# flanglet/kanzi-cpp

Measured on AMD Instinct MI355X. Metric: encode+decode MB/s on the synthetic stand-in for silesia.tar (bit-exact), higher is better.
Workload: dtype u8

## Files before the change

kanzi-cpp_amd/csrc/bwt_fwd.hip:

```cpp
#include "common.hpp"
#include "stages.hpp"
#include "bwt_common.hpp"

#include <cstdlib>
#include <cstring>
#include <algorithm>
#include <cmath>
#include "prims.hpp"
#include <chrono>
#include <vector>

namespace knz {

constexpr u32 SM_TS = 1792;
constexpr u32 SM_WIN = 2048;
constexpr u32 SM_G = 256;
constexpr u32 MED_CAP = 8192;
constexpr u32 MED_LO_CAP = 2048;
constexpr u32 SUPER_CAP = 8192;
constexpr int GATHER_THREADS = 512;
constexpr u32 GATHER_ROWS = 16;
static_assert(MED_CAP <= GATHER_ROWS * GATHER_THREADS, "k_bwt_f_gather_desc judges a medium group from one batch of loads");
constexpr u32 LARGE_OS_MIN = 1000000;
constexpr u32 NO_BIT = 0x7FFFFFFFu;
// ... 23 lines not shown

enum FwdCounter : u32 {
    CNT_SMALL_LEFT = 0,
    CNT_MED = 1,
    CNT_LARGE = 2,
    CNT_LARGE_MEMBERS = 3,
    CNT_RUN = 4,
    CNT_RUN_MEMBERS = 5,
    CNT_RUN_LONGEST = 6,
    CNT_SUPER = 7,
    CNT_RUNS = 8,
    CNT_MED_LO = 9,
    CNT_STAT_SMALL = 10,
    CNT_STAT_SMALL_GROUPS = 11,
    CNT_STAT_MED = 12,
    CNT_TIED = 13,
    CNT_PROBE_CAND = 14,
    CNT_LINKED = 14,
    CNT_LINK_TIED = 15,
    CNT_STAT_MED_GROUPS = 16,
    CNT_STAT_UNSPLIT = 17,
    CNT_STAT_UNSPLIT_MEMBERS = 18,
    CNT_STAT_MAJ = 19,
    CNT_STAT_MAJ_MEMBERS = 20,
    CNT_STAT_ASLEEP = 21,
    CNT_STAT_ASLEEP_MEMBERS = 22,
    CNT_RUN_TILES = 23,
    CNT_ROUND_SLOTS = 24,
    CNT_GAP_CLASSES = 25,
    CNT_GAP_MEMBERS = 26,
// ... 284 lines not shown
    __shared__ u32 inclAll[256];
    const int sgm = blockIdx.x, ps = blockIdx.y;
    const int tid = (int)threadIdx.x;
    u32* h = L.histAll + ((size_t)ps * L.nSeg + sgm) * 256;
    const u32 c = h[tid];
    u32 tot;
    const u32 incl = prims::sc_block_incl<prims::SCAN_SUM_EXCL>(c, wsum, &tot);
    inclAll[tid] = incl;
    __syncthreads();
    const bool last = ps + 1 == P;
    const u32 b0 = last ? base[sgm] : cbase[sgm];
    h[tid] = b0 + (tid ? inclAll[tid - 1] : 0u);
    if (last) gapStart[(size_t)sgm * 256 + tid] = b0 + incl - members[(size_t)sgm * 256 + tid];
}

__global__ __launch_bounds__(256) void k_bwt_f_r0_fill(u64* __restrict__ keys, const u32* __restrict__ members, const u32* __restrict__ gapStart,
                                                       const u32* __restrict__ firstPos, int P, int pbits)
{
    const u32 sgm = blockIdx.y;
    for (u32 c = 0; c < 256u; c++) {
        const u32 m = members[sgm * 256u + c];
        if (m == 0u) continue;
        const u32 g0 = gapStart[sgm * 256u + c];
        const u64 key = (rep_key(c, P) << pbits) | (u64)firstPos[sgm * 256u + c];
        for (u32 i = blockIdx.x * 256u + threadIdx.x; i < m; i += gridDim.x * 256u) keys[g0 + i] = key;
    }
}

constexpr u32 R0F_ROWS = 8;
__global__ __launch_bounds__(256) void k_bwt_f_r0_flags(const u64* __restrict__ keys, const u32* __restrict__ base, int nBlocks, u32 total, int P, int pbits,
                                                        unsigned long long* __restrict__ gbits64)
{
    __shared__ int sBlk;
    const u32 a0 = blockIdx.x * (256u * R0F_ROWS);
    if (threadIdx.x == 0) sBlk = find_block(base, nBlocks, a0 < total ? a0 : (total ? total - 1 : 0));
    __syncthreads();
    u64 kr[R0F_ROWS], kl[R0F_ROWS];
#pragma unroll
    for (u32 r = 0; r < R0F_ROWS; r++) {
        const u32 a = a0 + r * 256u + threadIdx.x;
        kr[r] = (a < total) ? keys[a] : 0ull;
        kl[r] = ((threadIdx.x & 63) == 0 && a > 0 && a < total) ? keys[a - 1] : 0ull;
    }
    int b = sBlk;
    const u64 pm = (1ull << pbits) - 1ull;
#pragma unroll
    for (u32 r = 0; r < R0F_ROWS; r++) {
        const u32 a = a0 + r * 256u + threadIdx.x;
        if (a0 + r * 256u >= total) break;
        const u64 k = kr[r];
        const u32 klo = (u32)__shfl_up((int)(u32)k, 1u, 64), khi = (u32)__shfl_up((int)(u32)(k >> 32), 1u, 64);
// ... 72 lines not shown
    const u32 word = W.bw[w];
    const u32 m = word & lowmask;
    int si = m ? (int)(w * 32 + 31 - __clz((int)m)) : W.prevSet[w];
    if (si < 0 || (u32)si >= SM_TS) return false;
    const u32 m2 = word & ~lowmask;
    const u32 ei = m2 ? (w * 32 + (u32)__ffs((int)m2) - 1) : W.nextSet[w];
    if (ei == NO_BIT) return false;
    const u32 len = ei - (u32)si;
    if (len < 2 || len > SM_G) return false;
    s = (u32)si; e = ei;
    return true;
}

__global__ __launch_bounds__(256) void k_bwt_f_r0_place_text(BwtView bv, FwdView v, const u32* __restrict__ winLastIncl, const u32* __restrict__ winFirstInclRev, u32 nWin,
                                                             uint2* __restrict__ largeNext, const u64* __restrict__ keys, int nsym, int pbits, uint2* __restrict__ runList,
                                                             const u32* __restrict__ gapTab)
{
    __shared__ SmWindow W;
    __shared__ int sBlk;
    __shared__ ClassAgg A;
    __shared__ u32 sSA[SM_WIN];
    __shared__ u64 sK[SM_WIN];
    __shared__ u32 sNew[64];
    __shared__ u32 sAfterLocal;
    constexpr int E = (int)(SM_WIN / 256);
    constexpr u32 TSW = SM_TS / 32;
    const int tid = (int)threadIdx.x;
    const u32 win = blockIdx.x;
    const u32 slot0 = win * SM_TS;
    if (tid == 0) sBlk = find_block(v.base, v.nBlocks, slot0 < v.total ? slot0 : v.total - 1);
    agg_init(A);
    if (tid < 64) {
        sNew[tid] = 0;
        const u32 w = v.gbits[(slot0 >> 5) + (u32)tid];
        W.bw[tid] = w;
        int pm = w ? (tid * 32 + 31 - __clz((int)w)) : -1;
        u32 sm = w ? (u32)(tid * 32 + __ffs((int)w) - 1) : NO_BIT;
        for (int o = 1; o < 64; o <<= 1) {
            const int t = __shfl_up(pm, (unsigned)o, 64);
            if (tid >= o) pm = t > pm ? t : pm;
            const u32 u = (u32)__shfl_down((int)sm, (unsigned)o, 64);
            if (tid + o < 64) sm = u < sm ? u : sm;
        }
        int pex = __shfl_up(pm, 1u, 64);
        if (tid == 0) pex = -1;
// ... 1683 lines not shown
static_assert(RUN_COLS == 4 * 256 && RUN_CH == 256 && RUN_ROWS % 4 == 0, "the kernels below map columns and rows to 256 threads");
static inline size_t run_tile_slots(size_t maxRuns) { return 2 * (maxRuns / RUN_TILE + 2); }

struct RunTile { u32 k0, k1, a, slot; bool first, last, multi; };
__device__ __forceinline__ RunTile run_tile(const u32* __restrict__ tileStart, const u32* __restrict__ segStart, u32 nRuns, u32 t)
{
    RunTile r;
    r.k0 = tileStart[t]; r.k1 = tileStart[t + 1]; r.a = segStart[r.k0];
    r.first = r.k0 == r.a;
    r.last = r.k1 >= nRuns || segStart[r.k1] == r.k1;
    r.multi = !(r.first && r.last);
    r.slot = (r.k1 - r.k0 == RUN_TILE) ? 2u * ((r.k0 + RUN_TILE - 1) / RUN_TILE) : (r.k0 >= RUN_TILE ? 2u * ((r.k0 - 1) / RUN_TILE) + 1u : 1u);
    return r;
}

__global__ __launch_bounds__(256) void k_bwt_f_run_seg_marks(const u64* __restrict__ sKey, u32 nRuns, int kbits, u32* __restrict__ segMark)
{
    const u32 k = blockIdx.x * 256 + threadIdx.x;
    if (k >= nRuns) return;
    segMark[k] = (k > 0 && (sKey[k] >> kbits) == (sKey[k - 1] >> kbits)) ? 0u : k;
}

__global__ __launch_bounds__(256) void k_bwt_f_run_tile_marks(const u32* __restrict__ segStart, u32 nRuns, u32* __restrict__ tileMark)
{
    const u32 k = blockIdx.x * 256 + threadIdx.x;
    if (k >= nRuns) return;
    tileMark[k] = ((k - segStart[k]) % RUN_TILE == 0) ? 1u : 0u;
}

__global__ __launch_bounds__(256) void k_bwt_f_run_tile_starts(const u32* __restrict__ segStart, const u32* __restrict__ tileIdx, u32 nRuns, u32* __restrict__ tileStart)
{
    const u32 k = blockIdx.x * 256 + threadIdx.x;
    if (k >= nRuns) return;
    const bool mark = (k - segStart[k]) % RUN_TILE == 0;
    const u32 t = tileIdx[k];
// ... 52 lines not shown
    }
    u32 run[4];
#pragma unroll
    for (u32 c = 0; c < 4; c++) run[c] = above ? carry - P[c] : P[c] - A[c];
    for (u32 t = t0; t < nT; t++) {
        const RunTile T = run_tile(tileStart, segStart, nRuns, t);
        u32* row = colTab + (size_t)T.slot * RUN_COLS;
#pragma unroll
        for (u32 c = 0; c < 4; c++) { const u32 x = row[tid + 256 * c]; row[tid + 256 * c] = run[c]; run[c] += x; }
        if (T.last) break;
    }
}

__global__ __launch_bounds__(256) void k_bwt_f_run_emit(const u32* __restrict__ tileStart, const u32* __restrict__ segStart, const u32* __restrict__ rcnt,
                                                        const u32* __restrict__ moff, const u64* __restrict__ sKey, const u32* __restrict__ sE, u32 nRuns, u32 M,
                                                        const u32* __restrict__ nTilesDev, const u32* __restrict__ colTab, u32 nsym, int kbits, int hbits,
                                                        u64* __restrict__ keys, u32* __restrict__ vals, u32* __restrict__ Rout)
{
    __shared__ u32 cnt[RUN_ROWS][RUN_CH];
    __shared__ u32 colBase[RUN_CH];
    __shared__ u32 wsum[4];
    __shared__ u32 sLmax;
    const u32 t = blockIdx.x, tid = threadIdx.x;
    if (t >= *nTilesDev) return;
    const int lane = lane_id();
    const u32 wave = tid >> 6;
    const RunTile T = run_tile(tileStart, segStart, nRuns, t);
    const u32 nRows = (T.k1 - T.k0 + 63) / 64;
    const u32 segBase = moff[T.a];
    const u32 tileMembers = (T.k1 < nRuns ? moff[T.k1] : M) - moff[T.k0];
    const bool above = ((sKey[T.k0] >> kbits) & 1ull) != 0;
    const u64 hiAll = (1ull << hbits) - 1ull;
    u32 Lr[RUN_ROWS / 4], rowMax[RUN_ROWS / 4], e[RUN_ROWS / 4];
    u64 kb[RUN_ROWS / 4];
    u32 lmax = 0;
    if (tid == 0) sLmax = 0;
#pragma unroll
    for (u32 q = 0; q < RUN_ROWS / 4; q++) {
        const u32 k = T.k0 + (wave + 4 * q) * 64 + (u32)lane;
        Lr[q] = 0; e[q] = 0; kb[q] = 0;
        if (k < T.k1) {
            const u64 key = sKey[k];
            Lr[q] = rcnt[k] + nsym - 1u;
            if (Lr[q] > RUN_DIRECT_LMAX) Lr[q] = RUN_DIRECT_LMAX;
            e[q] = sE[k];
            kb[q] = ((key >> (kbits + 1)) << (hbits + kbits)) | (key & ((1ull << kbits) - 1ull));
        }
        rowMax[q] = wave_max(Lr[q]);
        lmax = rowMax[q] > lmax ? rowMax[q] : lmax;
    }
    __syncthreads();
    if (lane == 0) atomicMax(&sLmax, lmax);
    __syncthreads();
    const u32 Lmax = sLmax;
    u32 carry = 0;
    for (u32 c0 = nsym; c0 <= Lmax; c0 += RUN_CH) {
        for (u32 i = tid; i < nRows * RUN_CH; i += 256) (&cnt[0][0])[i] = 0;
        __syncthreads();
#pragma unroll
        for (u32 q = 0; q < RUN_ROWS / 4; q++)
            if (Lr[q] >= c0) atomicAdd(&cnt[wave + 4 * q][Lr[q] - c0 < RUN_CH ? Lr[q] - c0 : RUN_CH - 1], 1u);
// ... 21 lines not shown
            const u32 P = carry + prims::sc_block_incl<prims::SCAN_SUM_EXCL>(colRuns, wsum, &tot);
            colBase[tid] = above ? tileMembers - P : P - colRuns;
            carry += tot;
        }
        __syncthreads();
#pragma unroll
        for (u32 q = 0; q < RUN_ROWS / 4; q++) {
            const u32 row = wave + 4 * q;
            if (row >= nRows) break;
            const u32 Rend = rowMax[q] < c0 + RUN_CH - 1 ? rowMax[q] : c0 + RUN_CH - 1;
            for (u32 R = c0; R <= Rend; R++) {
                const bool alive = Lr[q] >= R;
                const unsigned long long m = __ballot(alive);
                const u32 j = segBase + colBase[R - c0] + cnt[row][R - c0] + (u32)__popcll(m & __lanemask_lt());
                if (alive && j < M) {
                    keys[j] = kb[q] | ((above ? hiAll - (u64)R : (u64)R) << kbits);
                    vals[j] = e[q] - R;
                    Rout[j] = R;
                }
            }
        }
        __syncthreads();
    }
}

__global__ __launch_bounds__(256) void k_bwt_f_run_flags(const u64* __restrict__ keys, u32 M, unsigned long long* __restrict__ bits64)
{
    const u32 j = blockIdx.x * 256 + threadIdx.x;
    const u64 k = (j < M) ? keys[j] : 0ull;
    u32 klo = (u32)__shfl_up((int)(u32)k, 1u, 64), khi = (u32)__shfl_up((int)(u32)(k >> 32), 1u, 64);
    u64 kp = ((u64)khi << 32) | klo;
    if ((threadIdx.x & 63) == 0 && j > 0 && j < M) kp = keys[j - 1];
    const bool f = (j >= M) || (j == 0) || (k != kp);
    const unsigned long long m = __ballot(f);
    if ((threadIdx.x & 63) == 0) bits64[j >> 6] = m;
}

__global__ __launch_bounds__(256) void k_bwt_f_run_place(FwdView v, const uint2* __restrict__ desc, const u32* __restrict__ loff, u32 M, int kbits, const u64* __restrict__ keys,
                                                         const u32* __restrict__ vals, const u32* __restrict__ bits, const u32* __restrict__ winLastIncl,
                                                         const u32* __restrict__ winFirstInclRev, u32 nWin, uint2* __restrict__ largeNext, const u32* __restrict__ memberR,
                                                         u32* __restrict__ ovr, u32* __restrict__ rtbits, const u32* __restrict__ lbase, int allLabels)
{
    __shared__ SmWindow W;
    __shared__ ClassAgg A;
    const int tid = (int)threadIdx.x;
    const u32 jb = blockIdx.x * 256u;
    const u32 win = jb / SM_WIN, j0 = win * SM_WIN;
    agg_init(A);
    if (tid < 64) {
        const u32 w = bits[(j0 >> 5) + (u32)tid];
        W.bw[tid] = w;
        int pm = w ? (tid * 32 + 31 - __clz((int)w)) : -1;
        u32 sm = w ? (u32)(tid * 32 + __ffs((int)w) - 1) : NO_BIT;
        for (int o = 1; o < 64; o <<= 1) {
            const int t = __shfl_up(pm, (unsigned)o, 64);
            if (tid >= o) pm = t > pm ? t : pm;
            const u32 u = (u32)__shfl_down((int)sm, (unsigned)o, 64);
            if (tid + o < 64) sm = u < sm ? u : sm;
        }
        int pex = __shfl_up(pm, 1u, 64);
        if (tid == 0) pex = -1;
        u32 sex = (u32)__shfl_down((int)sm, 1u, 64);
        if (tid == 63) sex = NO_BIT;
// ... 1 lines not shown
        W.nextSet[tid] = sex;
    }
    __syncthreads();
    const u32 j = jb + (u32)tid;
    u32 surv = 0, mySlot = 0, hLocal = 0, hSize = 0;
    int hKind = -1;
    bool setBit = false;
    if (j < M) {
        const u32 i = j - j0;
        const u32 w = i >> 5, bit = i & 31;
        const u32 lowmask = (bit == 31) ? 0xFFFFFFFFu : ((2u << bit) - 1u);
        const u32 word = W.bw[w];
        const u32 m = word & lowmask;
        const int si = m ? (int)(w * 32 + 31 - (u32)__clz((int)m)) : W.prevSet[w];
        const u32 nh = (si >= 0) ? j0 + (u32)si : (win ? winLastIncl[win - 1] : 0u);
        const u32 di = (u32)(keys[j] >> kbits);
        const u32 gs = desc[di].x, off = loff[di];
        const u32 gp = vals[j];
        mySlot = gs + (j - off);
        v.SA[mySlot] = gp;
        if (nh != off || allLabels) lab_set(v, gp, lbase[di], gs + (nh - off), gs);
        ovr[mySlot] = memberR[j];
        if (nh == j) {
            const u32 m2 = word & ~lowmask;
            const u32 ei = m2 ? (w * 32 + (u32)__ffs((int)m2) - 1) : W.nextSet[w];
            u32 nxt = (ei != NO_BIT) ? j0 + ei : ((win + 1 < nWin) ? winFirstInclRev[nWin - 2 - win] : M);
            if (nxt > M) nxt = M;
            setBit = (j != off);
            hSize = nxt - j;
            hKind = agg_note(A, hSize, false, surv, hLocal);
        }
    }
    if (__ballot(surv != 0) != 0 && (tid & 63) == 0) v.counters[CNT_SMALL_LEFT] = 1;
    __syncthreads();
    if (tid == 0) agg_reserve(A, v);
    __syncthreads();
    if (hKind >= 0) agg_write(A, v, hKind, hLocal, mySlot, hSize, largeNext, (uint2*)nullptr);
    const int lane = tid & 63;
    const bool live = j < M;
    const u32 s0 = (u32)__shfl((int)mySlot, 0, 64);
    const bool inLine = live && (mySlot == s0 + (u32)lane);
    const unsigned long long hm = __ballot(setBit && inLine), rm = __ballot(inLine);
    if (live && !inLine) {
        if (setBit) atomicOr(&v.gnew[mySlot >> 5], 1u << (mySlot & 31));
        atomicOr(&rtbits[mySlot >> 5], 1u << (mySlot & 31));
    }
    if (lane == 0) {
        const u32 w0 = s0 >> 5, sh = s0 & 31;
        for (int which = 0; which < 2; which++) {
            const unsigned long long mask = which ? rm : hm;
            u32* dst = which ? rtbits : v.gnew;
            if (mask == 0) continue;
            const u32 p0 = (u32)(mask << sh);
            const u32 p1 = sh ? (u32)(mask >> (32 - sh)) : (u32)(mask >> 32);
            const u32 p2 = sh ? (u32)(mask >> (64 - sh)) : 0u;
            if (p0) atomicOr(&dst[w0], p0);
            if (p1) atomicOr(&dst[w0 + 1], p1);
            if (p2) atomicOr(&dst[w0 + 2], p2);
        }
    }
}

__global__ __launch_bounds__(256) void k_bwt_f_merge_bits(u32* __restrict__ gbits, u32* __restrict__ gnew, u32 nWords)
{
    const u32 w = blockIdx.x * 256 + threadIdx.x;
    if (w >= nWords) return;
    const u32 x = gnew[w];
    if (x) { gbits[w] |= x; gnew[w] = 0; }
}

__global__ __launch_bounds__(256) void k_bwt_f_emit(BwtView v, const u32* __restrict__ base, const u8* __restrict__ ok, const u32* __restrict__ SA,
                                                    FwdView fv, u32* __restrict__ newLen)
{
    const int b = blockIdx.y;
// ... 210 lines not shown
};

struct FwdSort {
    hipStream_t s; const XfStage& st; u32* hp;
    const FwdTuning tune = fwd_tuning();
    BwtView bv; FwdView v; FwdScratch w; size_t maxTotal;
    prims::RsWs rs1;
    u32 total, medSlots, nTiles; int nsym, pbits, kbits;
    bool groupSleep = false;
    u32 h = 1; int cur = 0;
    u64 *keysFree, *keysFree2;
    bool medFuse = false;
    bool runDirect = false;
    bool gaps = false;
    u32 gapClasses = 0, keptOut = 0, scanRuns = 0, scanLongest = 0;
    u32 nMedLo = 0;
    u32 nRun, runElems, surv, nMed, nLarge, largeElems, survMembers;
    LinkPlan link; LinkTrial linkTr; std::chrono::steady_clock::time_point statT;
    int fetch(u32 first, u32 n) { return hipMemcpyAsync(hp + first, w.counters + first, 4 * (size_t)n, hipMemcpyDeviceToHost, s) == hipSuccess && hipStreamSynchronize(s) == hipSuccess ? 0 : -1; }
    void merge_bits() { hipLaunchKernelGGL(k_bwt_f_merge_bits, GRID1(total / 32 + 2), w.gbits, w.gnew, total / 32 + 2); }
    void enable_run_tiebits() { if (!v.rtbits) { hipMemsetAsync(w.rtbits, 0, 4 * w.gbitsWords, s); v.ovr = w.ovr; v.rtbits = w.rtbits; } }
    void compact_medium(uint2* dst, u32 at = 0, u32 atLo = 0)
    {
        KScope ks_("k_bwt_f_med_compact");
        hipLaunchKernelGGL(k_bwt_f_med_flags, GRID1(medSlots), w.medStage, medSlots, w.medFlags);
        prims::launch_scan<prims::SCAN_SUM_EXCL>(s, w.medFlags, w.medPrefix, 2 * (size_t)medSlots, nullptr, w.scanTmp, w.counters + CNT_MED);
        hipLaunchKernelGGL(k_bwt_f_med_compact, GRID1(medSlots), w.medStage, medSlots, w.medPrefix, dst, at, w.medIdxLo, atLo, w.medIdxHi, at - atLo, w.counters + CNT_MED_LO);
    }
    void bounds(u32 n, bool last, const u32* bits = nullptr, u32 len = 0, u32 wordsPerWin = 0)
    {
// ... 74 lines not shown
        hipLaunchKernelGGL(k_bwt_f_r0_bases, dim3((unsigned)rs.L.nSeg, (unsigned)nsym), dim3(256), 0, s, rs.L, w.base, w.cbase, nsym, w.gapMembers, w.gapStart);
        for (int pass = 0; pass < nsym; pass++) {
            if (pass == 0) {
                TextSrcKept src; src.src = bv.src; src.P = nsym; src.pbits = pbits; src.shift = pbits; src.members = w.gapMembers;
                prims::rs_launch_pass_os<u64, false>(s, rs, src, nullptr, kout, nullptr, (size_t)bv.VS, pass);
                prims::rs_launch_layout(s, rsC);
            } else if (pass + 1 < nsym) {
                prims::DigitOfKey<u64> src; src.keys = kin; src.shift = pbits + 8 * pass; src.mask = 255u;
                prims::rs_launch_pass_os<u64, false>(s, rsC, src, nullptr, kout, nullptr, (size_t)bv.VS, pass);
            } else {
                LastPassSrc src; src.keys = kin; src.shift = pbits + 8 * pass; src.mask = 255u; src.members = w.gapMembers; src.gapStart = w.gapStart; src.P = nsym; src.pbits = pbits;
                prims::rs_launch_pass_os<u64, false>(s, rsC, src, nullptr, kout, nullptr, (size_t)bv.VS, pass);
            }
            std::swap(kin, kout);
        }
        hipLaunchKernelGGL(k_bwt_f_r0_fill, dim3(128, (unsigned)st.nBlocks), dim3(256), 0, s, kin, w.gapMembers, w.gapStart, w.gapFirst, nsym, pbits);
        keysFree = kout; keysFree2 = kin;
    }
    void round0_sort()
    {
        const prims::RsWs rs = prims::rs_carve(w.rsMem, maxTotal, st.nBlocks + 1, w.base, st.nBlocks);
        rs1 = prims::rs_carve(w.rsMem, maxTotal, st.nBlocks + 1, w.seg2, 1);
        { KScope ks_("k_bwt_f_r0_layout"); prims::rs_launch_layout(s, rs); }
        u64* kin = w.keysA; u64* kout = w.keysB;
        const bool oneRead = one_read();
        if (gaps) { round0_sort_gaps(rs); return; }
        if (oneRead) {
            KScope ks_("k_bwt_f_r0_sort");
            hipLaunchKernelGGL(k_bwt_f_r0_counts, dim3((unsigned)rs.L.nSeg), dim3(256), 0, s, bv, w.base, w.byteHist, nsym, rs.L, (const u32*)nullptr);
            hipLaunchKernelGGL(prims::k_rs_digit_bases, dim3((unsigned)rs.L.nSeg, (unsigned)nsym), dim3(256), 0, s, rs.L);
        }
// ... 2 lines not shown
            else prims::rs_launch_pass<u64, false>(s, rs, src, nullptr, kout, nullptr, (size_t)bv.VS);
        };
        for (int pass = 0; pass < nsym; pass++) {
            KScope ks_("k_bwt_f_r0_sort");
            if (pass == 0) { TextSrc src; src.src = bv.src; src.P = nsym; src.pbits = pbits; src.shift = pbits; sortPass(src, pass); }
            else { prims::DigitOfKey<u64> src; src.keys = kin; src.shift = pbits + 8 * pass; src.mask = 255u; sortPass(src, pass); }
            std::swap(kin, kout);
        }
        keysFree = kout; keysFree2 = kin;
    }
    int round0_place()
    {
        hipMemsetAsync(w.gbits, 0xFF, 4 * w.gbitsWords, s); hipMemsetAsync(w.gnew, 0, 4 * w.gbitsWords, s);
        hipMemsetAsync(w.counters, 0, 4 * CNT_ROUND_SLOTS, s);
        { KScope ks_("k_bwt_f_r0_flags"); hipLaunchKernelGGL(k_bwt_f_r0_flags, dim3((total + 256 * R0F_ROWS - 1) / (256 * R0F_ROWS)), dim3(256), 0, s, keysFree2, w.base, st.nBlocks, total, nsym, pbits,
                                                             reinterpret_cast<unsigned long long*>(w.gbits)); }
        bounds(nTiles, true, w.gbits, total, SM_TS / 32);
        kbits = bits_for((u64)bv.VS + 2, 1);
        const bool runRound = (2 * kbits + 1) < 64 && !tune.noRunRound;
        { KScope ks_("k_bwt_f_r0_place");
          hipLaunchKernelGGL(k_bwt_f_r0_place_text, dim3(nTiles), dim3(256), 0, s, bv, v, w.t1, w.t3, nTiles, w.large[cur], keysFree2, nsym, pbits, runRound ? w.runList : (uint2*)nullptr,
                             gaps ? w.classTab : (const u32*)nullptr);
          merge_bits(); }
        if (fetch(0, CNT_ROUND_SLOTS)) return -1;
        nRun = hp[CNT_RUN]; runElems = hp[CNT_RUN_MEMBERS];
        return 0;
    }
    int run_fallback()
    {
        { KScope ks_("k_bwt_f_run_fallback"); hipLaunchKernelGGL(k_bwt_f_run_fallback, GRID1(nRun), v, w.runList, nRun, w.med[cur], w.large[cur]); }
        nRun = 0; return fetch(0, CNT_ROUND_SLOTS);
    }
    int run_round()
    {
        if (nRun && ((u64)nRun > (1ull << (64 - (2 * kbits + 1))) || tune.runFallback) && run_fallback()) return -1;
        if (gaps) {
            if (nRun != gapClasses || runElems != keptOut) return -1;
            { KScope ks_("k_bwt_f_run_classes"); hipLaunchKernelGGL(k_bwt_f_run_classes, GRID1(nRun), bv, v, w.runList, nRun, w.classTab); }
            return run_round_sorted(scanRuns, scanLongest);
        }
// ... 12 lines not shown
        return run_round_sorted(hp[CNT_RUNS], hp[CNT_RUN_LONGEST]);
    }
    int run_round_sorted(const u32 nRuns, const u32 longest)
    {
        const int hbits = bits_for((u64)longest + 1, 1) + 1;
        const int rbits = bits_for(nRun, 0), idxBits = bits_for(nRuns, 1);
        if (nRuns == 0 || nRuns > w.maxRuns || rbits + hbits > 32 || idxBits + kbits + 1 + rbits > 64) return gaps ? -1 : run_fallback();
        { KScope ks_("k_bwt_f_large_prefix"); hipLaunchKernelGGL(k_bwt_f_large_prefix, dim3(1), dim3(1024), 0, s, w.runList, nRun, w.loff, w.base, st.nBlocks, w.lbase); }
        { KScope ks_("k_bwt_f_run_table"); hipLaunchKernelGGL(k_bwt_f_run_table, GRID1(nRuns), bv, v, w.runPos, nRuns, w.K, w.classTab, kbits, idxBits, w.runKeysA, w.runE, w.runL,
                                                              gaps ? w.runList : (const uint2*)nullptr, (u32)nsym); }
        const u64* rkSorted;
        { KScope ks_("k_bwt_f_sort_runs");
          rkSorted = sort_one_segment<u64, false>(nRuns, w.runKeysA, w.runKeysB, nullptr, nullptr, idxBits, idxBits + kbits + 1 + rbits) ? w.runKeysB : w.runKeysA; }
        { KScope ks_("k_bwt_f_run_sorted"); hipLaunchKernelGGL(k_bwt_f_run_sorted, GRID1(nRuns), rkSorted, nRuns, idxBits, w.runE, w.runL, (u32)nsym, w.sE, w.sKey, w.rcnt); }
        { KScope ks_("k_bwt_f_scan_sum"); prims::launch_scan<prims::SCAN_SUM_EXCL>(s, w.rcnt, w.moff, nRuns, nullptr, w.scanTmp); }
        u64* rk; u32* rv = w.valsA;
        runDirect = !tune.runSort && longest <= RUN_DIRECT_LMAX;
        if (runDirect) {
            KScope ks_("k_bwt_f_run_direct");
            u32* segStart = w.runPos; u32* tileIdx = w.runE;
            const u32 maxTiles = (u32)std::min<u64>((u64)nRuns, 2ull * nRun + nRuns / RUN_TILE + 1);
            hipLaunchKernelGGL(k_bwt_f_run_seg_marks, GRID1(nRuns), w.sKey, nRuns, kbits, segStart);
            prims::launch_scan<prims::SCAN_MAX_INCL>(s, segStart, segStart, nRuns, nullptr, w.scanTmp);
            hipLaunchKernelGGL(k_bwt_f_run_tile_marks, GRID1(nRuns), segStart, nRuns, tileIdx);
            prims::launch_scan<prims::SCAN_SUM_EXCL>(s, tileIdx, tileIdx, nRuns, nullptr, w.scanTmp, w.counters + CNT_RUN_TILES);
            hipLaunchKernelGGL(k_bwt_f_run_tile_starts, GRID1(nRuns), segStart, tileIdx, nRuns, w.runTileStart);
            if (nRuns > RUN_TILE) {
                hipLaunchKernelGGL(k_bwt_f_run_tile_counts, dim3(maxTiles), dim3(256), 0, s, w.runTileStart, segStart, w.rcnt, nRuns, w.counters + CNT_RUN_TILES, (u32)nsym, w.runColTab);
                hipLaunchKernelGGL(k_bwt_f_run_tile_scan, dim3(maxTiles), dim3(256), 0, s, w.runTileStart, segStart, w.sKey, nRuns, w.counters + CNT_RUN_TILES, (u32)nsym, kbits, w.runColTab);
            }
            rk = keysFree;
            hipLaunchKernelGGL(k_bwt_f_run_emit, dim3(maxTiles), dim3(256), 0, s, w.runTileStart, segStart, w.rcnt, w.moff, w.sKey, w.sE, nRuns, runElems, w.counters + CNT_RUN_TILES,
                               w.runColTab, (u32)nsym, kbits, hbits, rk, rv, w.valsB);
        } else {
            { KScope ks_("k_bwt_f_run_members"); hipLaunchKernelGGL(k_bwt_f_run_members, dim3((runElems + 2047) / 2048), dim3(256), 0, s, w.moff, nRuns, runElems, w.sKey, kbits, hbits,
                                                                    (u32)nsym, keysFree); }
            KScope ks_("k_bwt_f_sort_members");
            const int r = sort_one_segment<u64, false>(runElems, keysFree, keysFree2, nullptr, nullptr, 32, 32 + hbits + rbits);
            rk = r ? keysFree : keysFree2;
            hipLaunchKernelGGL(k_bwt_f_run_expand, GRID1(runElems), r ? keysFree2 : keysFree, runElems, w.sKey, w.sE, kbits, hbits, rk, rv, w.valsB);
        }
        u32* mbits = w.ebits; const u32 nWinM = (runElems + SM_WIN - 1) / SM_WIN;
        { KScope ks_("k_bwt_f_large_flags"); hipLaunchKernelGGL(k_bwt_f_run_flags, dim3(nWinM * (SM_WIN / 256)), dim3(256), 0, s, rk, runElems, reinterpret_cast<unsigned long long*>(mbits)); }
        bounds(nWinM, true, mbits, runElems, SM_WIN / 32);
        { KScope ks_("k_bwt_f_large_place");
          hipMemsetAsync(w.rtbits, 0, 4 * w.gbitsWords, s);
          hipLaunchKernelGGL(k_bwt_f_run_place, dim3((runElems + 255) / 256), dim3(256), 0, s, v, w.runList, w.loff, runElems, hbits + kbits, rk, rv, mbits, w.t1, w.t3, nWinM, w.large[cur],
                             w.valsB, w.ovr, w.rtbits, w.lbase, gaps ? 1 : 0);
          v.ovr = w.ovr; v.rtbits = w.rtbits; }
        { KScope ks_("k_bwt_f_merge_bits"); merge_bits(); }
        return 0;
    }
    int probe()
    {
        u32* probeCand = w.medFlags;
        compact_medium(w.med[cur]);
        { KScope ks_("k_bwt_f_probe"); hipLaunchKernelGGL(k_bwt_f_probe_scan, dim3(256), dim3(256), 0, s, v, w.med[cur], (u32)nsym, v.rtbits, probeCand); }
        if (fetch(0, CNT_ROUND_SLOTS)) return -1;
        surv = hp[CNT_SMALL_LEFT]; nMed = hp[CNT_MED]; nMedLo = hp[CNT_MED_LO]; nLarge = hp[CNT_LARGE]; largeElems = hp[CNT_LARGE_MEMBERS];
        if (const u32 nCand = hp[CNT_PROBE_CAND]) {
            enable_run_tiebits();
            hipMemsetAsync(w.counters, 0, 4 * CNT_PROBE_SLOTS, s);
            { KScope ks_("k_bwt_f_probe");
              hipLaunchKernelGGL(k_bwt_f_probe, dim3(std::min<u32>(nCand, 4096)), dim3(512), 0, s, bv, v, w.med[cur], probeCand, nCand, (u32)nsym, w.med[cur ^ 1], w.large[cur], w.ovr, w.rtbits);
              merge_bits(); }
            compact_medium(w.med[cur], nMed, nMedLo);
            if (fetch(0, CNT_MED_LO + 1)) return -1;
            surv |= hp[CNT_SMALL_LEFT]; nMed += hp[CNT_MED]; nMedLo += hp[CNT_MED_LO];
        }
        if (tune.stats) fprintf(stderr, "after round 0 (nsym %d, total %u): run groups %u (%u members); small left %u, medium %u, large %u (%u members); run members placed directly %u, sorted %u, kept out of the round-0 sort %u\n",
                                nsym, total, nRun, runElems, surv, nMed, nLarge, largeElems, (nRun && runDirect) ? runElems : 0u, (nRun && !runDirect) ? runElems : 0u, gaps ? keptOut : 0u);
        statT = std::chrono::steady_clock::now();
        return 0;
    }
    void link_step()
    {
        KScope ks_("k_bwt_f_link");
        u32* posflag = w.ebits; u32* linked = w.rbits; u32* rev = w.rcount; u32* sufRev = w.rprefix;
        const bool trial = link.mode == LinkPlan::TRIAL; linkTr.n = 0;
        if (trial) { linkTr.blk[linkTr.n++] = 0; if (st.nBlocks >= 5) linkTr.blk[linkTr.n++] = st.nBlocks / 2; if (st.nBlocks >= 3) linkTr.blk[linkTr.n++] = st.nBlocks - 1; }
        const u32 nW = total / 32 + 1;
        hipMemsetAsync(posflag, 0, 4 * (size_t)nW, s);
        hipMemsetAsync(linked, 0, 4 * ((size_t)nTiles * (SM_TS / 32) + 64), s);
        enable_run_tiebits();
        const u32 nTrial = (u32)std::min<u64>((u64)nTiles, ((u64)bv.VS + SM_TS - 1) / SM_TS + 2);
        const dim3 gridL(trial ? nTrial : nTiles, (unsigned)(linkTr.n ? linkTr.n : 1));
// ... 117 lines not shown
```

Measured before the change: 7424.

## Skip round-0 work inside gap interiors and emit run members directly into SA

Round-0 fill now writes keys only at the two margins of each large gap class. The flag and place kernels return early for workgroups that lie wholly inside a gap, clearing the gap's flag words instead of scanning keys. On the direct run path, the emit kernel now writes SA, ovr and a tie-flag byte straight to final slots, using string-mark and tie scans, rather than building keys and values. The place kernel is templated to find descriptors by binary search on loff. This removes full-key traffic and the run_flags pass, at the cost of extra scans, new kernels and more complex correctness conditions.

```diff
diff --git a/kanzi-cpp_amd/csrc/bwt_fwd.hip b/kanzi-cpp_amd/csrc/bwt_fwd.hip
--- a/kanzi-cpp_amd/csrc/bwt_fwd.hip
+++ b/kanzi-cpp_amd/csrc/bwt_fwd.hip
@@ -61,6 +61,7 @@
     CNT_STAT_SMALL = 10,
     CNT_STAT_SMALL_GROUPS = 11,
     CNT_STAT_MED = 12,
+    CNT_STAT_R0_SKIPPED = 12,
     CNT_TIED = 13,
     CNT_PROBE_CAND = 14,
     CNT_LINKED = 14,
@@ -375,27 +376,50 @@
     if (last) gapStart[(size_t)sgm * 256 + tid] = b0 + incl - members[(size_t)sgm * 256 + tid];
 }
 
+constexpr u32 R0F_ROWS = 8;
+constexpr u32 R0_GAP_MARGIN = 2048;
+static_assert(R0_GAP_MARGIN >= 256 * R0F_ROWS, "a workgroup of k_bwt_f_r0_flags that touches a gap's end must stay within the margin");
+static_assert(R0_GAP_MARGIN >= SM_WIN, "a window of k_bwt_f_r0_place_text that touches a gap's end must stay within the margin");
+
+__device__ __forceinline__ bool r0_inside_gap(const u32* __restrict__ members, const u32* __restrict__ gapStart, int b, u32 c, u32 a, u32 n)
+{
+    const u32 m = members[(u32)b * 256u + c];
+    if (m == 0u) return false;
+    const u32 g0 = gapStart[(u32)b * 256u + c];
+    return a > g0 && a - g0 < m && n <= m - (a - g0);
+}
+
 __global__ __launch_bounds__(256) void k_bwt_f_r0_fill(u64* __restrict__ keys, const u32* __restrict__ members, const u32* __restrict__ gapStart,
                                                        const u32* __restrict__ firstPos, int P, int pbits)
 {
-    const u32 sgm = blockIdx.y;
-    for (u32 c = 0; c < 256u; c++) {
-        const u32 m = members[sgm * 256u + c];
-        if (m == 0u) continue;
-        const u32 g0 = gapStart[sgm * 256u + c];
-        const u64 key = (rep_key(c, P) << pbits) | (u64)firstPos[sgm * 256u + c];
-        for (u32 i = blockIdx.x * 256u + threadIdx.x; i < m; i += gridDim.x * 256u) keys[g0 + i] = key;
-    }
-}
-
-constexpr u32 R0F_ROWS = 8;
+    const u32 sgm = blockIdx.y, c = blockIdx.x;
+    const u32 m = members[sgm * 256u + c];
+    if (m == 0u) return;
+    const u32 g0 = gapStart[sgm * 256u + c];
+    const u64 key = (rep_key(c, P) << pbits) | (u64)firstPos[sgm * 256u + c];
+    const bool whole = m <= 2u * R0_GAP_MARGIN;
+    const u32 cnt = whole ? m : 2u * R0_GAP_MARGIN;
+    for (u32 i = threadIdx.x; i < cnt; i += 256u) keys[g0 + ((whole || i < R0_GAP_MARGIN) ? i : m - 2u * R0_GAP_MARGIN + i)] = key;
+}
+
 __global__ __launch_bounds__(256) void k_bwt_f_r0_flags(const u64* __restrict__ keys, const u32* __restrict__ base, int nBlocks, u32 total, int P, int pbits,
-                                                        unsigned long long* __restrict__ gbits64)
+                                                        unsigned long long* __restrict__ gbits64, const u32* __restrict__ members, const u32* __restrict__ gapStart,
+                                                        u32* __restrict__ nSkipped)
 {
     __shared__ int sBlk;
+    __shared__ u32 sInside;
     const u32 a0 = blockIdx.x * (256u * R0F_ROWS);
-    if (threadIdx.x == 0) sBlk = find_block(base, nBlocks, a0 < total ? a0 : (total ? total - 1 : 0));
-    __syncthreads();
+    if (threadIdx.x == 0) { sBlk = find_block(base, nBlocks, a0 < total ? a0 : (total ? total - 1 : 0)); sInside = 0; }
+    __syncthreads();
+    if (members != nullptr) {
+        if (r0_inside_gap(members, gapStart, sBlk, threadIdx.x, a0, 256u * R0F_ROWS)) sInside = 1;
+        __syncthreads();
+        if (sInside) {
+            if (threadIdx.x < 256u * R0F_ROWS / 64u) gbits64[(a0 >> 6) + threadIdx.x] = 0ull;
+            if (nSkipped != nullptr && threadIdx.x == 0) atomicAdd(nSkipped, 1u);
+            return;
+        }
+    }
     u64 kr[R0F_ROWS], kl[R0F_ROWS];
 #pragma unroll
     for (u32 r = 0; r < R0F_ROWS; r++) {
@@ -498,7 +522,7 @@
 
 __global__ __launch_bounds__(256) void k_bwt_f_r0_place_text(BwtView bv, FwdView v, const u32* __restrict__ winLastIncl, const u32* __restrict__ winFirstInclRev, u32 nWin,
                                                              uint2* __restrict__ largeNext, const u64* __restrict__ keys, int nsym, int pbits, uint2* __restrict__ runList,
-                                                             const u32* __restrict__ gapTab)
+                                                             const u32* __restrict__ gapTab, const u32* __restrict__ gapMembers, const u32* __restrict__ gapStart)
 {
     __shared__ SmWindow W;
     __shared__ int sBlk;
@@ -507,12 +531,19 @@
     __shared__ u64 sK[SM_WIN];
     __shared__ u32 sNew[64];
     __shared__ u32 sAfterLocal;
+    __shared__ u32 sInside;
     constexpr int E = (int)(SM_WIN / 256);
     constexpr u32 TSW = SM_TS / 32;
     const int tid = (int)threadIdx.x;
     const u32 win = blockIdx.x;
     const u32 slot0 = win * SM_TS;
-    if (tid == 0) sBlk = find_block(v.base, v.nBlocks, slot0 < v.total ? slot0 : v.total - 1);
+    if (gapTab != nullptr) {
+        if (tid == 0) { sBlk = find_block(v.base, v.nBlocks, slot0 < v.total ? slot0 : v.total - 1); sInside = 0; }
+        __syncthreads();
+        if (r0_inside_gap(gapMembers, gapStart, sBlk, (u32)tid, slot0, SM_WIN)) sInside = 1;
+        __syncthreads();
+        if (sInside) return;
+    } else if (tid == 0) sBlk = find_block(v.base, v.nBlocks, slot0 < v.total ? slot0 : v.total - 1);
     agg_init(A);
     if (tid < 64) {
         sNew[tid] = 0;
@@ -2226,11 +2257,51 @@
     return r;
 }
 
-__global__ __launch_bounds__(256) void k_bwt_f_run_seg_marks(const u64* __restrict__ sKey, u32 nRuns, int kbits, u32* __restrict__ segMark)
+__global__ __launch_bounds__(256) void k_bwt_f_run_seg_marks(const u64* __restrict__ sKey, u32 nRuns, int kbits, u32* __restrict__ segMark, u32* __restrict__ strMark)
 {
     const u32 k = blockIdx.x * 256 + threadIdx.x;
     if (k >= nRuns) return;
-    segMark[k] = (k > 0 && (sKey[k] >> kbits) == (sKey[k - 1] >> kbits)) ? 0u : k;
+    const u64 key = sKey[k], prev = k > 0 ? sKey[k - 1] : 0ull;
+    segMark[k] = (k > 0 && (key >> kbits) == (prev >> kbits)) ? 0u : k;
+    strMark[k] = (k > 0 && key == prev) ? 0u : k;
+}
+
+constexpr int RUN_LBITS = 10;
+static_assert(RUN_DIRECT_LMAX < (1u << RUN_LBITS), "a run length of the direct path fits the low bits of tie[]");
+__global__ __launch_bounds__(256) void k_bwt_f_run_tie_marks(u32* __restrict__ tie, const u32* __restrict__ rcnt, u32 nRuns, u32 nsym)
+{
+    const u32 k = blockIdx.x * 256 + threadIdx.x;
+    if (k >= nRuns) return;
+    const u32 L = rcnt[k] + nsym - 1u;
+    tie[k] = (tie[k] << RUN_LBITS) | (L < (1u << RUN_LBITS) ? L : (1u << RUN_LBITS) - 1u);
+}
+
+__global__ __launch_bounds__(256) void k_bwt_f_run_tie_bits(const u8* __restrict__ flags, u32 M, u32 nWords, u32* __restrict__ mbits)
+{
+    const u32 w = blockIdx.x * 256 + threadIdx.x;
+    if (w >= nWords) return;
+    const u32 j0 = 32u * w;
+    u32 bits = 0;
+    if (j0 + 32u <= M) {
+        const u32x4 a = ldg<u32x4>(flags + j0), b = ldg<u32x4>(flags + j0 + 16);
+        const u32 x[8] = { a.x, a.y, a.z, a.w, b.x, b.y, b.z, b.w };
+#pragma unroll
+        for (u32 i = 0; i < 8; i++) bits |= ((x[i] * 0x00204081u) >> 21 & 0xFu) << (4 * i);
+    } else {
+        for (u32 i = 0; i < 32; i++) bits |= ((j0 + i >= M || flags[j0 + i] != 0) ? 1u : 0u) << i;
+    }
+    mbits[w] = bits;
+}
+
+__device__ __forceinline__ void or_mask64(u32* __restrict__ dst, u32 pos, unsigned long long mask)
+{
+    const u32 w0 = pos >> 5, sh = pos & 31;
+    const u32 p0 = (u32)(mask << sh);
+    const u32 p1 = sh ? (u32)(mask >> (32 - sh)) : (u32)(mask >> 32);
+    const u32 p2 = sh ? (u32)(mask >> (64 - sh)) : 0u;
+    if (p0) atomicOr(&dst[w0], p0);
+    if (p1) atomicOr(&dst[w0 + 1], p1);
+    if (p2) atomicOr(&dst[w0 + 2], p2);
 }
 
 __global__ __launch_bounds__(256) void k_bwt_f_run_tile_marks(const u32* __restrict__ segStart, u32 nRuns, u32* __restrict__ tileMark)
@@ -2313,8 +2384,9 @@
 
 __global__ __launch_bounds__(256) void k_bwt_f_run_emit(const u32* __restrict__ tileStart, const u32* __restrict__ segStart, const u32* __restrict__ rcnt,
                                                         const u32* __restrict__ moff, const u64* __restrict__ sKey, const u32* __restrict__ sE, u32 nRuns, u32 M,
-                                                        const u32* __restrict__ nTilesDev, const u32* __restrict__ colTab, u32 nsym, int kbits, int hbits,
-                                                        u64* __restrict__ keys, u32* __restrict__ vals, u32* __restrict__ Rout)
+                                                        const u32* __restrict__ nTilesDev, const u32* __restrict__ colTab, u32 nsym, int kbits,
+                                                        const uint2* __restrict__ desc, const u32* __restrict__ loff, const u32* __restrict__ tie,
+                                                        u32* __restrict__ SA, u32* __restrict__ ovr, u8* __restrict__ flags)
 {
     __shared__ u32 cnt[RUN_ROWS][RUN_CH];
     __shared__ u32 colBase[RUN_CH];
@@ -2326,24 +2398,24 @@
     const u32 wave = tid >> 6;
     const RunTile T = run_tile(tileStart, segStart, nRuns, t);
     const u32 nRows = (T.k1 - T.k0 + 63) / 64;
+    const u32 tileMembers = (T.k1 < nRuns ? moff[T.k1] : M) - moff[T.k0];
+    const u64 key0 = sKey[T.k0];
+    const bool above = ((key0 >> kbits) & 1ull) != 0;
+    const u32 di = (u32)(key0 >> (kbits + 1));
     const u32 segBase = moff[T.a];
-    const u32 tileMembers = (T.k1 < nRuns ? moff[T.k1] : M) - moff[T.k0];
-    const bool above = ((sKey[T.k0] >> kbits) & 1ull) != 0;
-    const u64 hiAll = (1ull << hbits) - 1ull;
-    u32 Lr[RUN_ROWS / 4], rowMax[RUN_ROWS / 4], e[RUN_ROWS / 4];
-    u64 kb[RUN_ROWS / 4];
+    const u32 slotBase = desc[di].x - loff[di];
+    u32 Lr[RUN_ROWS / 4], rowMax[RUN_ROWS / 4], e[RUN_ROWS / 4], Pr[RUN_ROWS / 4];
     u32 lmax = 0;
     if (tid == 0) sLmax = 0;
 #pragma unroll
     for (u32 q = 0; q < RUN_ROWS / 4; q++) {
         const u32 k = T.k0 + (wave + 4 * q) * 64 + (u32)lane;
-        Lr[q] = 0; e[q] = 0; kb[q] = 0;
+        Lr[q] = 0; e[q] = 0; Pr[q] = 0;
         if (k < T.k1) {
-            const u64 key = sKey[k];
             Lr[q] = rcnt[k] + nsym - 1u;
             if (Lr[q] > RUN_DIRECT_LMAX) Lr[q] = RUN_DIRECT_LMAX;
             e[q] = sE[k];
-            kb[q] = ((key >> (kbits + 1)) << (hbits + kbits)) | (key & ((1ull << kbits) - 1ull));
+            if ((tie[k] >> RUN_LBITS) != k) Pr[q] = tie[k - 1] & ((1u << RUN_LBITS) - 1u);
         }
         rowMax[q] = wave_max(Lr[q]);
         lmax = rowMax[q] > lmax ? rowMax[q] : lmax;
@@ -2395,9 +2467,10 @@
                 const unsigned long long m = __ballot(alive);
                 const u32 j = segBase + colBase[R - c0] + cnt[row][R - c0] + (u32)__popcll(m & __lanemask_lt());
                 if (alive && j < M) {
-                    keys[j] = kb[q] | ((above ? hiAll - (u64)R : (u64)R) << kbits);
-                    vals[j] = e[q] - R;
-                    Rout[j] = R;
+                    const u32 mySlot = slotBase + j;
+                    SA[mySlot] = e[q] - R;
+                    ovr[mySlot] = R;
+                    flags[j] = R > Pr[q] ? 1 : 0;
                 }
             }
         }
@@ -2417,17 +2490,25 @@
     if ((threadIdx.x & 63) == 0) bits64[j >> 6] = m;
 }
 
-__global__ __launch_bounds__(256) void k_bwt_f_run_place(FwdView v, const uint2* __restrict__ desc, const u32* __restrict__ loff, u32 M, int kbits, const u64* __restrict__ keys,
-                                                         const u32* __restrict__ vals, const u32* __restrict__ bits, const u32* __restrict__ winLastIncl,
-                                                         const u32* __restrict__ winFirstInclRev, u32 nWin, uint2* __restrict__ largeNext, const u32* __restrict__ memberR,
-                                                         u32* __restrict__ ovr, u32* __restrict__ rtbits, const u32* __restrict__ lbase, int allLabels)
+template <bool DIRECT>
+__global__ __launch_bounds__(256) void k_bwt_f_run_place(FwdView v, const uint2* __restrict__ desc, const u32* __restrict__ loff, u32 nDesc, u32 M, int kbits,
+                                                         const u64* __restrict__ keys, const u32* __restrict__ vals, const u32* __restrict__ bits,
+                                                         const u32* __restrict__ winLastIncl, const u32* __restrict__ winFirstInclRev, u32 nWin,
+                                                         uint2* __restrict__ largeNext, const u32* __restrict__ memberR, u32* __restrict__ ovr,
+                                                         u32* __restrict__ rtbits, const u32* __restrict__ lbase, int allLabels)
 {
     __shared__ SmWindow W;
     __shared__ ClassAgg A;
+    __shared__ u32 sDi;
     const int tid = (int)threadIdx.x;
     const u32 jb = blockIdx.x * 256u;
     const u32 win = jb / SM_WIN, j0 = win * SM_WIN;
     agg_init(A);
+    if (DIRECT && tid == 64) {
+        u32 lo = 0, hi = nDesc;
+        while (hi - lo > 1) { const u32 mid = (lo + hi) >> 1; if (loff[mid] <= jb) lo = mid; else hi = mid; }
+        sDi = lo;
+    }
     if (tid < 64) {
         const u32 w = bits[(j0 >> 5) + (u32)tid];
         W.bw[tid] = w;
@@ -2459,13 +2540,15 @@
         const u32 m = word & lowmask;
         const int si = m ? (int)(w * 32 + 31 - (u32)__clz((int)m)) : W.prevSet[w];
         const u32 nh = (si >= 0) ? j0 + (u32)si : (win ? winLastIncl[win - 1] : 0u);
-        const u32 di = (u32)(keys[j] >> kbits);
+        u32 di;
+        if (DIRECT) { di = sDi; while (di + 1 < nDesc && j >= loff[di + 1]) di++; }
+        else di = (u32)(keys[j] >> kbits);
         const u32 gs = desc[di].x, off = loff[di];
-        const u32 gp = vals[j];
         mySlot = gs + (j - off);
-        v.SA[mySlot] = gp;
+        const u32 gp = DIRECT ? v.SA[mySlot] : vals[j];
+        if (!DIRECT) v.SA[mySlot] = gp;
         if (nh != off || allLabels) lab_set(v, gp, lbase[di], gs + (nh - off), gs);
-        ovr[mySlot] = memberR[j];
+        if (!DIRECT) ovr[mySlot] = memberR[j];
         if (nh == j) {
             const u32 m2 = word & ~lowmask;
             const u32 ei = m2 ? (w * 32 + (u32)__ffs((int)m2) - 1) : W.nextSet[w];
@@ -2491,18 +2574,8 @@
         atomicOr(&rtbits[mySlot >> 5], 1u << (mySlot & 31));
     }
     if (lane == 0) {
-        const u32 w0 = s0 >> 5, sh = s0 & 31;
-        for (int which = 0; which < 2; which++) {
-            const unsigned long long mask = which ? rm : hm;
-            u32* dst = which ? rtbits : v.gnew;
-            if (mask == 0) continue;
-            const u32 p0 = (u32)(mask << sh);
-            const u32 p1 = sh ? (u32)(mask >> (32 - sh)) : (u32)(mask >> 32);
-            const u32 p2 = sh ? (u32)(mask >> (64 - sh)) : 0u;
-            if (p0) atomicOr(&dst[w0], p0);
-            if (p1) atomicOr(&dst[w0 + 1], p1);
-            if (p2) atomicOr(&dst[w0 + 2], p2);
-        }
+        if (hm) or_mask64(v.gnew, s0, hm);
+        if (rm) or_mask64(rtbits, s0, rm);
     }
 }
 
@@ -2743,6 +2816,7 @@
     bool runDirect = false;
     bool gaps = false;
     u32 gapClasses = 0, keptOut = 0, scanRuns = 0, scanLongest = 0;
+    u32 r0Skipped = 0;
     u32 nMedLo = 0;
     u32 nRun, runElems, surv, nMed, nLarge, largeElems, survMembers;
     LinkPlan link; LinkTrial linkTr; std::chrono::steady_clock::time_point statT;
@@ -2847,7 +2921,7 @@
             }
             std::swap(kin, kout);
         }
-        hipLaunchKernelGGL(k_bwt_f_r0_fill, dim3(128, (unsigned)st.nBlocks), dim3(256), 0, s, kin, w.gapMembers, w.gapStart, w.gapFirst, nsym, pbits);
+        hipLaunchKernelGGL(k_bwt_f_r0_fill, dim3(256, (unsigned)st.nBlocks), dim3(256), 0, s, kin, w.gapMembers, w.gapStart, w.gapFirst, nsym, pbits);
         keysFree = kout; keysFree2 = kin;
     }
     void round0_sort()
@@ -2880,16 +2954,17 @@
         hipMemsetAsync(w.gbits, 0xFF, 4 * w.gbitsWords, s); hipMemsetAsync(w.gnew, 0, 4 * w.gbitsWords, s);
         hipMemsetAsync(w.counters, 0, 4 * CNT_ROUND_SLOTS, s);
         { KScope ks_("k_bwt_f_r0_flags"); hipLaunchKernelGGL(k_bwt_f_r0_flags, dim3((total + 256 * R0F_ROWS - 1) / (256 * R0F_ROWS)), dim3(256), 0, s, keysFree2, w.base, st.nBlocks, total, nsym, pbits,
-                                                             reinterpret_cast<unsigned long long*>(w.gbits)); }
+                                                             reinterpret_cast<unsigned long long*>(w.gbits), gaps ? w.gapMembers : (const u32*)nullptr, w.gapStart,
+                                                             tune.stats ? w.counters + CNT_STAT_R0_SKIPPED : (u32*)nullptr); }
         bounds(nTiles, true, w.gbits, total, SM_TS / 32);
         kbits = bits_for((u64)bv.VS + 2, 1);
         const bool runRound = (2 * kbits + 1) < 64 && !tune.noRunRound;
         { KScope ks_("k_bwt_f_r0_place");
           hipLaunchKernelGGL(k_bwt_f_r0_place_text, dim3(nTiles), dim3(256), 0, s, bv, v, w.t1, w.t3, nTiles, w.large[cur], keysFree2, nsym, pbits, runRound ? w.runList : (uint2*)nullptr,
-                             gaps ? w.classTab : (const u32*)nullptr);
+                             gaps ? w.classTab : (const u32*)nullptr, w.gapMembers, w.gapStart);
           merge_bits(); }
         if (fetch(0, CNT_ROUND_SLOTS)) return -1;
-        nRun = hp[CNT_RUN]; runElems = hp[CNT_RUN_MEMBERS];
+        nRun = hp[CNT_RUN]; runElems = hp[CNT_RUN_MEMBERS]; r0Skipped = hp[CNT_STAT_R0_SKIPPED];
         return 0;
     }
     int run_fallback()
@@ -2932,14 +3007,19 @@
           rkSorted = sort_one_segment<u64, false>(nRuns, w.runKeysA, w.runKeysB, nullptr, nullptr, idxBits, idxBits + kbits + 1 + rbits) ? w.runKeysB : w.runKeysA; }
         { KScope ks_("k_bwt_f_run_sorted"); hipLaunchKernelGGL(k_bwt_f_run_sorted, GRID1(nRuns), rkSorted, nRuns, idxBits, w.runE, w.runL, (u32)nsym, w.sE, w.sKey, w.rcnt); }
         { KScope ks_("k_bwt_f_scan_sum"); prims::launch_scan<prims::SCAN_SUM_EXCL>(s, w.rcnt, w.moff, nRuns, nullptr, w.scanTmp); }
-        u64* rk; u32* rv = w.valsA;
-        runDirect = !tune.runSort && longest <= RUN_DIRECT_LMAX;
+        u64* rk = nullptr; u32* rv = w.valsA;
+        u32* mbits = w.ebits; const u32 nWinM = (runElems + SM_WIN - 1) / SM_WIN;
+        runDirect = !tune.runSort && longest <= RUN_DIRECT_LMAX && idxBits + RUN_LBITS <= 32;
         if (runDirect) {
             KScope ks_("k_bwt_f_run_direct");
-            u32* segStart = w.runPos; u32* tileIdx = w.runE;
+            u32* segStart = w.runPos; u32* tileIdx = w.runE; u32* tie = w.runL;
+            u8* flags = reinterpret_cast<u8*>(keysFree);
             const u32 maxTiles = (u32)std::min<u64>((u64)nRuns, 2ull * nRun + nRuns / RUN_TILE + 1);
-            hipLaunchKernelGGL(k_bwt_f_run_seg_marks, GRID1(nRuns), w.sKey, nRuns, kbits, segStart);
+            hipLaunchKernelGGL(k_bwt_f_run_seg_marks, GRID1(nRuns), w.sKey, nRuns, kbits, segStart, tie);
             prims::launch_scan<prims::SCAN_MAX_INCL>(s, segStart, segStart, nRuns, nullptr, w.scanTmp);
+            prims::launch_scan<prims::SCAN_MAX_INCL>(s, tie, tie, nRuns, nullptr, w.scanTmp);
+            hipLaunchKernelGGL(k_bwt_f_run_tie_marks, GRID1(nRuns), tie, w.rcnt, nRuns, (u32)nsym);
+            prims::launch_scan<prims::SCAN_MAX_INCL>(s, tie, tie, nRuns, nullptr, w.scanTmp);
             hipLaunchKernelGGL(k_bwt_f_run_tile_marks, GRID1(nRuns), segStart, nRuns, tileIdx);
             prims::launch_scan<prims::SCAN_SUM_EXCL>(s, tileIdx, tileIdx, nRuns, nullptr, w.scanTmp, w.counters + CNT_RUN_TILES);
             hipLaunchKernelGGL(k_bwt_f_run_tile_starts, GRID1(nRuns), segStart, tileIdx, nRuns, w.runTileStart);
@@ -2947,24 +3027,28 @@
                 hipLaunchKernelGGL(k_bwt_f_run_tile_counts, dim3(maxTiles), dim3(256), 0, s, w.runTileStart, segStart, w.rcnt, nRuns, w.counters + CNT_RUN_TILES, (u32)nsym, w.runColTab);
                 hipLaunchKernelGGL(k_bwt_f_run_tile_scan, dim3(maxTiles), dim3(256), 0, s, w.runTileStart, segStart, w.sKey, nRuns, w.counters + CNT_RUN_TILES, (u32)nsym, kbits, w.runColTab);
             }
-            rk = keysFree;
             hipLaunchKernelGGL(k_bwt_f_run_emit, dim3(maxTiles), dim3(256), 0, s, w.runTileStart, segStart, w.rcnt, w.moff, w.sKey, w.sE, nRuns, runElems, w.counters + CNT_RUN_TILES,
-                               w.runColTab, (u32)nsym, kbits, hbits, rk, rv, w.valsB);
+                               w.runColTab, (u32)nsym, kbits, w.runList, w.loff, tie, w.SA, w.ovr, flags);
+            hipLaunchKernelGGL(k_bwt_f_run_tie_bits, GRID1(nWinM * (SM_WIN / 32)), flags, runElems, nWinM * (SM_WIN / 32), mbits);
         } else {
             { KScope ks_("k_bwt_f_run_members"); hipLaunchKernelGGL(k_bwt_f_run_members, dim3((runElems + 2047) / 2048), dim3(256), 0, s, w.moff, nRuns, runElems, w.sKey, kbits, hbits,
                                                                     (u32)nsym, keysFree); }
-            KScope ks_("k_bwt_f_sort_members");
-            const int r = sort_one_segment<u64, false>(runElems, keysFree, keysFree2, nullptr, nullptr, 32, 32 + hbits + rbits);
-            rk = r ? keysFree : keysFree2;
-            hipLaunchKernelGGL(k_bwt_f_run_expand, GRID1(runElems), r ? keysFree2 : keysFree, runElems, w.sKey, w.sE, kbits, hbits, rk, rv, w.valsB);
-        }
-        u32* mbits = w.ebits; const u32 nWinM = (runElems + SM_WIN - 1) / SM_WIN;
-        { KScope ks_("k_bwt_f_large_flags"); hipLaunchKernelGGL(k_bwt_f_run_flags, dim3(nWinM * (SM_WIN / 256)), dim3(256), 0, s, rk, runElems, reinterpret_cast<unsigned long long*>(mbits)); }
+            { KScope ks_("k_bwt_f_sort_members");
+              const int r = sort_one_segment<u64, false>(runElems, keysFree, keysFree2, nullptr, nullptr, 32, 32 + hbits + rbits);
+              rk = r ? keysFree : keysFree2;
+              hipLaunchKernelGGL(k_bwt_f_run_expand, GRID1(runElems), r ? keysFree2 : keysFree, runElems, w.sKey, w.sE, kbits, hbits, rk, rv, w.valsB); }
+            KScope ks_("k_bwt_f_large_flags");
+            hipLaunchKernelGGL(k_bwt_f_run_flags, dim3(nWinM * (SM_WIN / 256)), dim3(256), 0, s, rk, runElems, reinterpret_cast<unsigned long long*>(mbits));
+        }
         bounds(nWinM, true, mbits, runElems, SM_WIN / 32);
         { KScope ks_("k_bwt_f_large_place");
           hipMemsetAsync(w.rtbits, 0, 4 * w.gbitsWords, s);
-          hipLaunchKernelGGL(k_bwt_f_run_place, dim3((runElems + 255) / 256), dim3(256), 0, s, v, w.runList, w.loff, runElems, hbits + kbits, rk, rv, mbits, w.t1, w.t3, nWinM, w.large[cur],
-                             w.valsB, w.ovr, w.rtbits, w.lbase, gaps ? 1 : 0);
+          if (runDirect)
+              hipLaunchKernelGGL(k_bwt_f_run_place<true>, dim3((runElems + 255) / 256), dim3(256), 0, s, v, w.runList, w.loff, nRun, runElems, hbits + kbits, (const u64*)nullptr,
+                                 (const u32*)nullptr, mbits, w.t1, w.t3, nWinM, w.large[cur], (const u32*)nullptr, w.ovr, w.rtbits, w.lbase, gaps ? 1 : 0);
+          else
+              hipLaunchKernelGGL(k_bwt_f_run_place<false>, dim3((runElems + 255) / 256), dim3(256), 0, s, v, w.runList, w.loff, nRun, runElems, hbits + kbits, rk, rv, mbits, w.t1, w.t3,
+                                 nWinM, w.large[cur], w.valsB, w.ovr, w.rtbits, w.lbase, gaps ? 1 : 0);
           v.ovr = w.ovr; v.rtbits = w.rtbits; }
         { KScope ks_("k_bwt_f_merge_bits"); merge_bits(); }
         return 0;
@@ -2986,8 +3070,9 @@
             if (fetch(0, CNT_MED_LO + 1)) return -1;
             surv |= hp[CNT_SMALL_LEFT]; nMed += hp[CNT_MED]; nMedLo += hp[CNT_MED_LO];
         }
-        if (tune.stats) fprintf(stderr, "after round 0 (nsym %d, total %u): run groups %u (%u members); small left %u, medium %u, large %u (%u members); run members placed directly %u, sorted %u, kept out of the round-0 sort %u\n",
-                                nsym, total, nRun, runElems, surv, nMed, nLarge, largeElems, (nRun && runDirect) ? runElems : 0u, (nRun && !runDirect) ? runElems : 0u, gaps ? keptOut : 0u);
+        if (tune.stats) fprintf(stderr, "after round 0 (nsym %d, total %u): run groups %u (%u members); small left %u, medium %u, large %u (%u members); run members placed directly %u, sorted %u, kept out of the round-0 sort %u; flag workgroups inside a gap %u\n",
+                                nsym, total, nRun, runElems, surv, nMed, nLarge, largeElems, (nRun && runDirect) ? runElems : 0u, (nRun && !runDirect) ? runElems : 0u, gaps ? keptOut : 0u,
+                                gaps ? r0Skipped : 0u);
         statT = std::chrono::steady_clock::now();
         return 0;
     }
```

Result: faster. 7757 (median of 6 runs) (+4.5%).
